# Aazmp/vp8oclenc

Hardware: AMD Instinct MI355X
Metric: macroblocks/sec inter-frame (ME+DCT+loopfilter), 1080p (higher is better)
Workload: dtype u8/int32

## Files before the change

vp8oclenc_amd/build.py:

```python
from __future__ import annotations

import os
import shutil
import subprocess

PKG = os.path.dirname(os.path.abspath(__file__))
CSRC = os.path.join(PKG, "csrc")
LIB = os.path.join(PKG, "libvp8hip.so")
SOURCES = ["api_context.hip", "api_intake.hip", "api_inter.hip", "api_entropy.hip", "api_batch.hip", "api_shard.hip", "api_profile.hip", "kernels_me.hip", "kernels_scale.hip", "kernels_denoise.hip", "api_denoise.hip", "kernels_analysis.hip", "api_analysis.hip", "kernels_convert.hip", "kernels_deinterlace.hip", "api_deinterlace.hip", "kernels_geometry.hip", "api_geometry.hip", "kernels_s2.hip", "kernels_mb.hip", "kernels_lf3.hip", "kernels_lf4.hip", "kernels_lf_simple.hip", "kernels_quality.hip", "api_quality.hip", "kernels_entropy_stage.hip", "kernels_rc.hip", "kernels_intra.hip", "vp8_host.cpp", "vp8_driver.cpp", "vp8_bitstream.cpp"]
HEADERS = ["vp8hip_ctx.h", "vp8hip_dev.h", "kernels_rc_dev.h", "lf_shared.h", "lf_banded.h", "lds_bank_model.h", "s1_pre_layout.h", "vp8_rfc6386_tables.inc", "vp8_mbhdr.h", "kernels_ent.hip", "kernels_hdr.hip"]
HEADERS = HEADERS + [os.path.join("..", "..", "include", h) for h in ("vp8hip.h", "vp8hip_multi.h", "vp8hip_taps.h", "vp8hip_host.h", "vp8hip_driver.h", "vp8hip_bitstream.h")]


def _hipcc() -> str:
    for cand in (shutil.which("hipcc"), "/opt/rocm/bin/hipcc"):
        if cand and os.path.exists(cand):
            return cand
    raise RuntimeError("hipcc not found: the MI355X path cannot be built (there is no CPU fallback)")


def stale() -> bool:
    if not os.path.exists(LIB):
        return True
    t = os.path.getmtime(LIB)
    deps = [os.path.join(CSRC, s) for s in SOURCES] + [os.path.normpath(os.path.join(CSRC, h)) for h in HEADERS]
    return any(os.path.exists(d) and os.path.getmtime(d) > t for d in deps)


def build(force: bool = False, verbose: bool = False) -> str:
    if not force and not stale():
        return LIB
    objs = []
    procs = []
    odir = os.path.join(PKG, "build")
    os.makedirs(odir, exist_ok=True)
    flags = ["--offload-arch=gfx950", "-O3", "-fPIC", "-std=c++17", "-ffp-contract=off", "-Wall", "-Wno-unused-function", "-Wno-bitwise-instead-of-logical", "-Wno-unused-value", "-Wno-missing-braces",
             "-I", os.path.join(PKG, "..", "include")] + os.environ.get("VP8HIP_EXTRA_FLAGS", "").split()
    for src in SOURCES:
        path = os.path.join(CSRC, src)
        if not os.path.exists(path):
            continue
        obj = os.path.join(odir, os.path.splitext(src)[0] + ".o")
        objs.append(obj)
# ... 20 lines not shown
```

vp8oclenc_amd/csrc/api_profile.hip:

```cpp
#include "vp8hip_ctx.h"

using namespace vp8;

namespace vp8 {

int prof_collect(vp8hip_ctx *c) {
    if (c->ev_used == 0) return VP8HIP_OK;
    HIPCHK(c, hipStreamSynchronize(c->stream));
    for (int i = 0; i < c->ev_used; i += 2) {
        float ms = 0;
        HIPCHK(c, hipEventElapsedTime(&ms, c->ev[i], c->ev[i + 1]));
        c->prof_ms[c->ev_kernel[i / 2]] += ms;
        c->prof_n[c->ev_kernel[i / 2]] += 1;
    }
    c->ev_used = 0;
    return VP8HIP_OK;
}

}

extern "C" {

int vp8hip_profile_enable(vp8hip_ctx *c, uint32_t mask) {
    USE_DEVICE(c);
// ... 109 lines not shown
    HIPCHK(c, hipStreamSynchronize(s));
    return VP8HIP_OK;
}

int vp8hip_debug_weight(vp8hip_ctx *c, const int32_t *d, int n, int32_t *out) {
    USE_DEVICE(c);
    JOIN_LF(c);
    if (!c || !d || !out || n <= 0) return VP8HIP_ERR_ARG;
    int32_t *dd = nullptr, *dout = nullptr;
    HIPCHK(c, hipMalloc(&dd, (size_t)n * 64));
    HIPCHK(c, hipMalloc(&dout, (size_t)n * 4));
    HIPCHK(c, hipMemcpyAsync(dd, d, (size_t)n * 64, hipMemcpyHostToDevice, c->stream));
    launch_weight_tap(c->stream, dd, n, dout);
    HIPCHK(c, hipMemcpyAsync(out, dout, (size_t)n * 4, hipMemcpyDeviceToHost, c->stream));
    HIPCHK(c, hipStreamSynchronize(c->stream));
    hipFree(dd);
    hipFree(dout);
    return VP8HIP_OK;
}

int vp8hip_debug_weight_mfma(vp8hip_ctx *c, const int32_t *d, int n, int32_t *out) {
    USE_DEVICE(c);
    JOIN_LF(c);
    if (!c || !d || !out || n <= 0) return VP8HIP_ERR_ARG;
    int32_t *dd = nullptr, *dout = nullptr;
    HIPCHK(c, hipMalloc(&dd, (size_t)n * 64));
    HIPCHK(c, hipMalloc(&dout, (size_t)n * 4));
    HIPCHK(c, hipMemcpyAsync(dd, d, (size_t)n * 64, hipMemcpyHostToDevice, c->stream));
    launch_weight_tap_mfma(c->stream, dd, n, dout);
    HIPCHK(c, hipMemcpyAsync(out, dout, (size_t)n * 4, hipMemcpyDeviceToHost, c->stream));
    HIPCHK(c, hipStreamSynchronize(c->stream));
    hipFree(dd);
    hipFree(dout);
    return VP8HIP_OK;
}

int vp8hip_debug_lf_stall(vp8hip_ctx *c, int on) {
    USE_DEVICE(c);
    JOIN_LF(c);
    if (!c) return VP8HIP_ERR_ARG;
    c->lf_stall_test = on ? 1 : 0;
    return VP8HIP_OK;
}

int vp8hip_debug_upload_ssim(vp8hip_ctx *c, const float *ssim) {
    USE_DEVICE(c);
    JOIN_LF(c);
    if (!c || !ssim) return VP8HIP_ERR_ARG;
    HIPCHK(c, hipMemcpyAsync(c->out.ssim, ssim, (size_t)c->mbs * 4, hipMemcpyHostToDevice, c->stream));
    HIPCHK(c, hipStreamSynchronize(c->stream));
    return VP8HIP_OK;
}

int vp8hip_debug_upload_header_inputs(vp8hip_ctx *c, const int32_t *seg, const int32_t *nz, const int32_t *ref, const int32_t *parts,
                                      const int16_t *vectors, const int32_t *is_inter, const int32_t *modes, const uint32_t *probs,
                                      const uint32_t *denom, const int32_t *sd) {
    USE_DEVICE(c);
    JOIN_LF(c);
    if (!c) return VP8HIP_ERR_ARG;
    hipStream_t s = c->stream;
    const size_t n = c->mbs;
    if (seg) HIPCHK(c, hipMemcpyAsync(c->out.seg, seg, n * 4, hipMemcpyHostToDevice, s));
    if (nz) HIPCHK(c, hipMemcpyAsync(c->out.nz, nz, n * 4, hipMemcpyHostToDevice, s));
    if (ref) HIPCHK(c, hipMemcpyAsync(c->out.ref, ref, n * 4, hipMemcpyHostToDevice, s));
    if (parts) HIPCHK(c, hipMemcpyAsync(c->out.parts, parts, n * 4, hipMemcpyHostToDevice, s));
    if (vectors) HIPCHK(c, hipMemcpyAsync(c->out.vec, vectors, n * 16, hipMemcpyHostToDevice, s));
// ... 12 lines not shown
```

vp8oclenc_amd/csrc/kernels_me.hip:

```cpp
#include <stdlib.h>
#include <string.h>

#include "vp8hip_dev.h"
#include "s1_pre_layout.h"

namespace vp8 {

struct BorderItem { Plane y, u, v; };
static_assert(EXT == 8, "border_row stores a margin as one eight-byte word");
__device__ __forceinline__ void border_row(const Plane &pl, int row, int lane) {
    if (row >= pl.h + EXT) return;
    uint8_t *dst = pl.p + (ptrdiff_t)row * pl.stride;
    const uint8_t *src = pl.p + (ptrdiff_t)iclamp(row, 0, pl.h - 1) * pl.stride;
    if (row < 0 || row >= pl.h)
        for (int x = lane * 8; x < pl.w; x += 512) *reinterpret_cast<uint2 *>(dst + x) = *reinterpret_cast<const uint2 *>(src + x);
    if (lane < 2) {
        const uint32_t s4 = (uint32_t)src[lane ? pl.w - 1 : 0] * 0x01010101u;
        *reinterpret_cast<uint2 *>(dst + (lane ? pl.w : -EXT)) = make_uint2(s4, s4);
    }
}
__device__ __forceinline__ void border_body(const BorderItem &a) {
    border_row(blockIdx.y == 0 ? a.y : (blockIdx.y == 1 ? a.u : a.v), (int)blockIdx.x - EXT, threadIdx.x);
}

__global__ __launch_bounds__(64) void k_border(BorderItem a) { border_body(a); }

void launch_border(hipStream_t s, const Frame &f) {
    dim3 grid(f.Y[0].h + 2 * EXT, 3);
    VP8_LAUNCH(k_border, grid, dim3(64), 0, s, BorderItem{f.Y[0], f.U, f.V});
}

struct PyrArgs { Frame f[2 * MAX_BATCH]; uint32_t border_mask; };
static int border_jobs(const Frame &f) { return (f.Y[0].h + 2 * EXT) + 2 * (f.U.h + 2 * EXT); }

__global__ __launch_bounds__(256) void k_pyramid(PyrArgs a) {
    __shared__ uint8_t s2[16][16];
    __shared__ uint8_t s3[8][8];
// ... 139 lines not shown
    int refmap[3];
    int nrefs;
    int net_width, w, h, pixel_rate, rate_shift, nblk, bw;
    int pbw, pbh;
    uint32_t bw_inv;
};

template <bool SPLIT>
struct S1Map {
    static constexpr int LANES_PER_BLOCK = SPLIT ? 20 : 5;
    static constexpr int BLOCKS_PER_WAVE = SPLIT ? 3 : 12;
    static constexpr int BLOCKS_PER_WG = 4 * BLOCKS_PER_WAVE;
};

__device__ __forceinline__ void s1_subblock(const uint8_t *cp, int cstride, const uint8_t *rp, int rstride, int acc[5]) {
    uint32_t c[4], q0[4], q1[4];
#pragma unroll
    for (int y = 0; y < 4; ++y) {
        c[y] = *reinterpret_cast<const uint32_t *>(cp + (ptrdiff_t)y * cstride) ^ 0x80808080u;
        const uint2 q = ld_u64(rp + (ptrdiff_t)y * rstride);
        q0[y] = q.x ^ 0x80808080u; q1[y] = q.y ^ 0x80808080u;
    }
    uint32_t cc[4], col[8];
    transpose4x4(c, cc);
    transpose4x4(q0, col);
    transpose4x4(q1, col + 4);
    int pre[16];
#pragma unroll
    for (int k = 0; k < 4; ++k) weight_pre_column(cc[k], pre + 4 * k);
#pragma unroll
    for (int i = 0; i < 5; ++i) acc[i] += weight_cols_pre(pre, col + i);
}

__device__ __forceinline__ int vcopy(uint32_t x) {
    int y;
    asm volatile("v_mov_b32 %0, %1" : "=v"(y) : "v"(x));
    return y;
}
__device__ __forceinline__ void s1_subblock_pre(v4i wa, const int *pre_lds, int pre_off, const uint8_t *rp, int rstride, int acc[5]) {
    uint32_t q0[4], q1[4];
#pragma unroll
    for (int y = 0; y < 4; ++y) {
        const uint2 q = ld_u64(rp + (ptrdiff_t)y * rstride);
        q0[y] = q.x ^ 0x80808080u; q1[y] = q.y ^ 0x80808080u;
    }
    uint32_t col[8];
    transpose4x4(q0, col);
    transpose4x4(q1, col + 4);
#pragma unroll
    for (int i = 0; i < 5; ++i) {
        int off = pre_off;
        asm volatile("" : "+v"(off));
        __builtin_amdgcn_sched_barrier(0);
        const v4i b = (i & 1) ? v4i{vcopy(col[i]), vcopy(col[i + 1]), vcopy(col[i + 2]), vcopy(col[i + 3])}
                              : v4i{(int)col[i], (int)col[i + 1], (int)col[i + 2], (int)col[i + 3]};
        acc[i] += weight_mfma(wa, load_pre16(pre_lds + off), b);
    }
}
static_assert(s1_pre_c_read_worst() == 4 && s1_pre_c_read_best() == 4, "the C reads of the whole-pel search's pre table must be free of LDS bank conflicts");
static_assert(S1_PRE_BLOCKS == S1Map<false>::BLOCKS_PER_WAVE, "s1_pre_layout.h and the loop form's lane map disagree");
__device__ __forceinline__ void s1_make_pre(const Plane &cur, int cx, int cy, int sb, bool on, int *dst16) {
    const int sx = (sb >> 1) * 4, sy = (sb & 1) * 4;
    const uint8_t *cp = cur.p + (ptrdiff_t)(cy + sy) * cur.stride + cx + sx;
    uint32_t c[4], cc[4];
#pragma unroll
    for (int y = 0; y < 4; ++y) c[y] = *reinterpret_cast<const uint32_t *>(cp + (ptrdiff_t)y * cur.stride) ^ 0x80808080u;
    transpose4x4(c, cc);
    int pre[16];
    weight_pre_block(cc, pre);
    if (on) {
#pragma unroll
        for (int k = 0; k < 4; ++k) *reinterpret_cast<int4 *>(dst16 + 4 * k) = make_int4(pre[4 * k], pre[4 * k + 1], pre[4 * k + 2], pre[4 * k + 3]);
    }
}

template <bool SPLIT, bool PRE_LDS = false>
__device__ __forceinline__ uint32_t search1_block(const Search1Args &a, int r, int cx, int cy, uint32_t pv, bool live, int sub, int lane,
                                                  const int *pre_lds = nullptr ,
                                                  int pre_off = 0 ) {
    const int sb0 = sub / 5, j = sub - 5 * sb0;
    int v0x = (int16_t)(pv & 0xffffu), v0y = (int16_t)(pv >> 16);
    const int rmask = a.pixel_rate - 1;
    v0x = (v0x + ((v0x >> 31) & rmask)) >> a.rate_shift;
    v0y = (v0y + ((v0y >> 31) & rmask)) >> a.rate_shift;
    if (a.pixel_rate > 8) v0x = v0y = 0;

    const int py = (int16_t)(cy + v0y + (j - 2));
    const bool row_valid = live && py >= 0 && py <= a.h - 8;
    const int xb = cx + v0x - 2;
    const bool loadable = row_valid && xb >= -8 && xb <= a.w - 4;
    const int lx = loadable ? xb : cx, ly = loadable ? py : cy;

    const uint8_t *cp = a.cur.p + (ptrdiff_t)cy * a.cur.stride + cx;
    const uint8_t *rp = a.ref[r].p + (ptrdiff_t)ly * a.ref[r].stride + lx;
    int acc[5] = {0, 0, 0, 0, 0};
    if (SPLIT) {
        const int sx = (sb0 >> 1) * 4, sy = (sb0 & 1) * 4;
        s1_subblock(cp + (ptrdiff_t)sy * a.cur.stride + sx, a.cur.stride, rp + (ptrdiff_t)sy * a.ref[r].stride + sx, a.ref[r].stride, acc);
#pragma unroll
        for (int i = 0; i < 5; ++i) {
            acc[i] += __shfl(acc[i], lane + 10, 64);
            acc[i] += __shfl(acc[i], lane + 5, 64);
        }
    } else {
        if (PRE_LDS) {
            const v4i wa = metric_a(lane);
#pragma unroll 1
            for (int sb = 0; sb < 4; ++sb) {
                const int sx = (sb >> 1) * 4, sy = (sb & 1) * 4;
                s1_subblock_pre(wa, pre_lds, pre_off + s1_pre_sub_at(sb), rp + (ptrdiff_t)sy * a.ref[r].stride + sx, a.ref[r].stride, acc);
            }
        } else {
#pragma unroll 1
            for (int sb = 0; sb < 4; ++sb) {
                const int sx = (sb >> 1) * 4, sy = (sb & 1) * 4;
                s1_subblock(cp + (ptrdiff_t)sy * a.cur.stride + sx, a.cur.stride, rp + (ptrdiff_t)sy * a.ref[r].stride + sx, a.ref[r].stride, acc);
            }
        }
    }
    const int pen_mask = a.pixel_rate < 4 ? -1 : 0;
    const int pen_y = iabs(iabs(py - cy) - v0y);
    uint32_t best = 0xffffffffu;
#pragma unroll
    for (int i = 0; i < 5; ++i) {
        const int px = (int16_t)(xb + i);
        const bool valid = loadable && px >= 0 && px <= a.w - 8;
        const int diff = (acc[i] + (((iabs(iabs(px - cx) - v0x) + pen_y) << 5) & pen_mask)) & 0xffff;
        const uint32_t key = (valid && diff < 0x7fff) ? ((uint32_t)diff << 8) | (uint32_t)(j * 5 + i) : 0xffffffffu;
        best = key < best ? key : best;
    }
#pragma unroll
    for (int off = 1; off <= 4; off <<= 1) {
        const uint32_t o = (uint32_t)__shfl((int)best, lane + off, 64);
        if (j + off < 5 && o < best) best = o;
    }
    int bx, by;
    if (best != 0xffffffffu) {
        const int k = best & 0xff;
        bx = v0x + (k % 5 - 2);
        by = v0y + (k / 5 - 2);
    } else {
        bx = (int16_t)(v0x - cx);
        by = (int16_t)(v0y - cy);
    }
    const uint32_t ox16 = (uint16_t)(int16_t)((int16_t)bx * (int16_t)a.pixel_rate);
    const uint32_t oy16 = (uint16_t)(int16_t)((int16_t)by * (int16_t)a.pixel_rate);
    return ox16 | (oy16 << 16);
}

template <bool SPLIT, bool PRE_LDS = false, bool REF_LOOP = false>
__device__ __forceinline__ void search1_body(const Search1Args &a) {
    using M = S1Map<SPLIT>;
    if (!REF_LOOP && (int)blockIdx.y >= a.nrefs) return;
    const int lane = threadIdx.x & 63, wave = threadIdx.x >> 6;
    const int grp = lane / M::LANES_PER_BLOCK, sub = lane - M::LANES_PER_BLOCK * grp;
    const int b_raw = (xcd_band(blockIdx.x, gridDim.x) * 4 + wave) * M::BLOCKS_PER_WAVE + grp;
    const bool live = grp < M::BLOCKS_PER_WAVE && b_raw < a.nblk;
    const int b = live ? b_raw : a.nblk - 1;
    const int by = a.bw == 1 ? b : (int)__umulhi((uint32_t)b, a.bw_inv), bx = b - by * a.bw;
    const int cx = bx * 8, cy = by * 8;
    const int parent = (cy >> 4) * a.net_width + (cx >> 4);
    const bool parent_written = (cx >> 4) < a.pbw && (cy >> 4) < a.pbh;
    const int *pre_lds = nullptr;
    int pre_off = 0;
    if (!SPLIT && PRE_LDS) {
        __shared__ __attribute__((aligned(16))) int s_pre[4][S1_PRE_INTS];
        const int slot = lane >> 2, sb = lane & 3;
        const int tb_raw = (xcd_band(blockIdx.x, gridDim.x) * 4 + wave) * M::BLOCKS_PER_WAVE + slot;
        const int tb = tb_raw < a.nblk ? tb_raw : a.nblk - 1;
        const int tby = a.bw == 1 ? tb : (int)__umulhi((uint32_t)tb, a.bw_inv), tbx = tb - tby * a.bw;
        s1_make_pre(a.cur, tbx * 8, tby * 8, sb, slot < M::BLOCKS_PER_WAVE, &s_pre[0][0] + s1_pre_slot_at(wave, slot) + s1_pre_sub_at(sb));
        asm volatile("s_waitcnt lgkmcnt(0)" ::: "memory");
        pre_lds = &s_pre[0][0];
        pre_off = s1_pre_c_at(wave, lane, 0, 0);
    }
    const int nr = REF_LOOP ? a.nrefs : 1;
#pragma unroll 1
    for (int ri = 0; ri < nr; ++ri) {
        const int r = a.refmap[REF_LOOP ? ri : (int)blockIdx.y];
        const uint32_t pv = parent_written ? reinterpret_cast<const uint32_t *>(a.src[r])[parent] : 0u;
        const uint32_t out = search1_block<SPLIT, !SPLIT && PRE_LDS>(a, r, cx, cy, pv, live, sub, lane, pre_lds, pre_off);
        if (sub == 0 && live) {
            const int cell = (cy >> 3) * a.net_width + (cx >> 3);
            reinterpret_cast<uint32_t *>(a.dst[r])[cell] = out;
        }
    }
}

struct CoarseArgs { Search1Args lv[5]; };
constexpr int COARSE_WAVES = 6;
template <bool FINEST, bool TOP_ONLY = false>
__device__ __forceinline__ void coarse_tile(const Search1Args &L0, const Search1Args &L1, const Search1Args &L2, const Search1Args &L3, const Search1Args &L4, int r) {
    using M = S1Map<true>;
    __shared__ uint32_t mv4, mv3, mv2[4], mv1[16];
    const int lane = threadIdx.x & 63, wave = threadIdx.x >> 6;
    const int grp = lane / M::LANES_PER_BLOCK, sub = lane - M::LANES_PER_BLOCK * grp;
    const int slot = grp < M::BLOCKS_PER_WAVE ? wave * M::BLOCKS_PER_WAVE + grp : 99;
    const int tiles_x = (L1.bw + 3) / 4;
    const int tile = xcd_band(blockIdx.x, gridDim.x);
    const int ty = tile / tiles_x, tx = tile - ty * tiles_x;
    {
        const int bx = tx >> 1, by = ty >> 1;
        const bool exists = bx < L4.bw && by * L4.bw + bx < L4.nblk;
        if (wave == 0) {
            const bool live = slot == 0 && exists;
            const uint32_t out = search1_block<true>(L4, r, (live ? bx : 0) * 8, (live ? by : 0) * 8, 0u, live, sub, lane);
            if (slot == 0 && sub == 0) mv4 = exists ? out : 0u;
        }
    }
    __syncthreads();
    {
        const bool exists = tx < L3.bw && ty * L3.bw + tx < L3.nblk;
        if (wave == 0) {
            const bool live = slot == 0 && exists;
// ... 60 lines not shown
    s.net_width = a.net_width;
    s.w = g.w;
    s.h = g.h;
    s.pixel_rate = 1 << l;
    s.rate_shift = l;
    s.bw = g.w / 8;
    s.nblk = (g.w / 8) * (g.h / 8);
    return s;
}
__global__ __launch_bounds__(128) void k_search1_top_b(CoarseBatchArgs a) {
    const CoarseMember &m = a.m[blockIdx.z];
    if ((int)blockIdx.y >= m.nrefs) return;
    const int r = m.refmap[blockIdx.y];
    const Search1Args L1 = coarse_level(a, m, 1, r), L2 = coarse_level(a, m, 2, r), L3 = coarse_level(a, m, 3, r), L4 = coarse_level(a, m, 4, r);
    coarse_tile<false, true>(L1, L1, L2, L3, L4, 0);
}
template <bool FINEST>
__global__ __launch_bounds__(64 * COARSE_WAVES) void k_search1_coarse_b(CoarseBatchArgs a) {
    const CoarseMember &m = a.m[blockIdx.z];
    if ((int)blockIdx.y >= m.nrefs) return;
    const int r = m.refmap[blockIdx.y];
    const Search1Args L0 = coarse_level(a, m, 0, r), L1 = coarse_level(a, m, 1, r), L2 = coarse_level(a, m, 2, r), L3 = coarse_level(a, m, 3, r),
                      L4 = coarse_level(a, m, 4, r);
    coarse_tile<FINEST>(L0, L1, L2, L3, L4, 0);
}

template <bool SPLIT>
__global__ __launch_bounds__(256) void k_search1(Search1Args a) { search1_body<SPLIT>(a); }
static_assert(sizeof(BatchOf<Search1Args>) <= 4096 && sizeof(PyrArgs) <= 4096 && sizeof(BatchOf<PackItem>) <= 4096, "a batch's argument blocks travel in the 4 KiB kernel-argument segment");
template <bool SPLIT>
__global__ __launch_bounds__(256) void k_search1_b(BatchOf<Search1Args> b) { search1_body<SPLIT>(b.item[blockIdx.z]); }
__global__ __attribute__((amdgpu_waves_per_eu(8, 8))) __launch_bounds__(256) void k_search1_pl(Search1Args a) { search1_body<false, true>(a); }
__global__ __attribute__((amdgpu_waves_per_eu(8, 8))) __launch_bounds__(256) void k_search1_pl_b(BatchOf<Search1Args> b) { search1_body<false, true>(b.item[blockIdx.z]); }
__global__ __attribute__((amdgpu_waves_per_eu(7, 8))) __launch_bounds__(256) void k_search1_plr_b(BatchOf<Search1Args> b) { search1_body<false, true, true>(b.item[blockIdx.z]); }
static bool search1_ref_loop() {
    static const bool on = [] { const char *v = getenv("VP8HIP_S1_REF_LOOP"); return !(v && v[0] == '0'); }();
    return on;
}
static bool search1_pre_lds() {
    static const bool on = [] { const char *v = getenv("VP8HIP_S1_PRE_LDS"); return !(v && v[0] == '0'); }();
    return on;
}

static Search1Args search1_args(const CodingItem &it, int level, int src_idx, int net_width) {
    const Frame &cur = *it.cur;
    const RefSet &refs = it.refs;
    const NetSet &nets = *it.nets;
    Search1Args a;
    a.cur = cur.Y[level];
    int n = 0;
    for (int r = 0; r < 3; ++r) {
        a.ref[r] = refs.ref[r].Y[level];
        a.src[r] = nets.net[r][src_idx];
        a.dst[r] = nets.net[r][src_idx ^ 1];
        if (refs.use[r]) a.refmap[n++] = r;
    }
    a.nrefs = n;
    for (int i = n; i < 3; ++i) a.refmap[i] = 0;
    a.net_width = net_width;
    a.w = a.cur.w;
    a.h = a.cur.h;
    a.pixel_rate = 1 << level;
    a.rate_shift = level;
    a.bw = a.w / 8;
    a.nblk = (a.w / 8) * (a.h / 8);
    a.bw_inv = a.bw > 0 ? (uint32_t)(((1ull << 32) + a.bw - 1) / a.bw) : 0;
    a.pbw = level < 4 ? cur.Y[level + 1].w / 8 : 0;
// ... 64 lines not shown
            if (refs.use[r]) m.refmap[k++] = r;
        }
        m.nrefs = k;
        for (int j = k; j < 3; ++j) m.refmap[j] = 0;
        maxrefs = k > maxrefs ? k : maxrefs;
    }
    const int bw0 = a.g[0].w / 8, bh0 = a.g[0].h / 8, bw1 = a.g[1].w / 8, bh1 = a.g[1].h / 8;
    if (bw0 * bh0 <= 0 || maxrefs == 0 || search1_skip()) return true;
    const int tiles_x = finest ? (bw0 + 7) / 8 : (bw1 + 3) / 4, tiles_y = finest ? (bh0 + 7) / 8 : (bh1 + 3) / 4;
    if (tiles_x * tiles_y <= 0) return !finest ? true : false;
    if (top_only) {
        VP8_LAUNCH(k_search1_top_b, dim3(tiles_x * tiles_y, maxrefs, n), dim3(128), 0, s, a);
        return true;
    }
    if (finest) VP8_LAUNCH(k_search1_coarse_b<true>, dim3(tiles_x * tiles_y, maxrefs, n), dim3(64 * COARSE_WAVES), 0, s, a);
    else VP8_LAUNCH(k_search1_coarse_b<false>, dim3(tiles_x * tiles_y, maxrefs, n), dim3(64 * COARSE_WAVES), 0, s, a);
    return true;
}

void launch_search1_batch(hipStream_t s, const CodingItem *items, int n, int level, int src_idx, int net_width) {
    BatchOf<Search1Args> b;
    b.n = n;
    int maxrefs = 0, totrefs = 0;
    for (int i = 0; i < n; ++i) {
        b.item[i] = search1_args(items[i], level, src_idx, net_width);
        maxrefs = b.item[i].nrefs > maxrefs ? b.item[i].nrefs : maxrefs;
        totrefs += b.item[i].nrefs;
    }
    const int nblk = b.item[0].nblk;
    if (nblk <= 0 || maxrefs == 0 || search1_skip()) return;
    if (search1_split((size_t)nblk * totrefs, false))
        VP8_LAUNCH(k_search1_b<true>, dim3((nblk + S1Map<true>::BLOCKS_PER_WG - 1) / S1Map<true>::BLOCKS_PER_WG, maxrefs, n), dim3(256), 0, s, b);
    else if (search1_pre_lds() && search1_ref_loop())
        VP8_LAUNCH(k_search1_plr_b, dim3((nblk + S1Map<false>::BLOCKS_PER_WG - 1) / S1Map<false>::BLOCKS_PER_WG, 1, n), dim3(256), 0, s, b);
    else if (search1_pre_lds())
        VP8_LAUNCH(k_search1_pl_b, dim3((nblk + S1Map<false>::BLOCKS_PER_WG - 1) / S1Map<false>::BLOCKS_PER_WG, maxrefs, n), dim3(256), 0, s, b);
    else
        VP8_LAUNCH(k_search1_b<false>, dim3((nblk + S1Map<false>::BLOCKS_PER_WG - 1) / S1Map<false>::BLOCKS_PER_WG, maxrefs, n), dim3(256), 0, s, b);
}

__global__ __launch_bounds__(256) void k_weight_tap(const int32_t *d, int n, int32_t *out) {
    const int i = blockIdx.x * 256 + threadIdx.x;
    if (i >= n) return;
    uint32_t cc[4], pp[4];
#pragma unroll
    for (int c = 0; c < 4; ++c) {
        cc[c] = pp[c] = 0;
#pragma unroll
        for (int r = 0; r < 4; ++r) {
            const int v = d[i * 16 + 4 * r + c];
            const uint32_t cb = (uint32_t)(v > 0 ? v : 0) ^ 0x80u, pb = (uint32_t)(v > 0 ? 0 : -v) ^ 0x80u;
            cc[c] |= cb << (8 * r);
            pp[c] |= pb << (8 * r);
        }
    }
    int pre[16];
#pragma unroll
    for (int c = 0; c < 4; ++c) weight_pre_column(cc[c], pre + 4 * c);
    out[i] = weight_cols_pre(pre, pp);
}
void launch_weight_tap(hipStream_t s, const int32_t *d, int n, int32_t *out) {
    hipLaunchKernelGGL(k_weight_tap, dim3((n + 255) / 256), dim3(256), 0, s, d, n, out);
}
__global__ __attribute__((amdgpu_waves_per_eu(8, 8))) __launch_bounds__(256) void k_weight_tap_mfma(const int32_t *d, int n, int32_t *out) {
    const int i0 = blockIdx.x * 256 + threadIdx.x, i = i0 < n ? i0 : n - 1;
    uint32_t cc[4];
    v4i pp;
#pragma unroll
    for (int c = 0; c < 4; ++c) {
        uint32_t cw = 0, pw = 0;
#pragma unroll
        for (int r = 0; r < 4; ++r) {
            const int v = d[i * 16 + 4 * r + c];
            const uint32_t cb = (uint32_t)(v > 0 ? v : 0) ^ 0x80u, pb = (uint32_t)(v > 0 ? 0 : -v) ^ 0x80u;
            cw |= cb << (8 * r);
            pw |= pb << (8 * r);
        }
        cc[c] = cw;
        pp[c] = (int)pw;
    }
    int pre[16];
    weight_pre_block(cc, pre);
    v16i c16;
#pragma unroll
    for (int k = 0; k < 16; ++k) c16[k] = pre[k];
    const int w = weight_mfma(metric_a((int)threadIdx.x), c16, pp);
    if (i0 < n) out[i0] = w;
}
void launch_weight_tap_mfma(hipStream_t s, const int32_t *d, int n, int32_t *out) {
    hipLaunchKernelGGL(k_weight_tap_mfma, dim3((n + 255) / 256), dim3(256), 0, s, d, n, out);
}

}
```

vp8oclenc_amd/csrc/vp8hip_dev.h:

```cpp
#pragma once
#include <hip/hip_runtime.h>
#include <hip/hip_ext.h>
#include <stdint.h>
#include <stdlib.h>
#include <string.h>

#include <vector>

#include "../../include/vp8hip.h"

namespace vp8 {

struct LaunchTiming { hipEvent_t start = nullptr, stop = nullptr; int launches = 0; };
extern thread_local LaunchTiming tl_timing;
#define VP8_LAUNCH(kernel, grid, block, shmem, stream, ...)                                                                               \
    do {                                                                                                                                  \
        ++::vp8::tl_timing.launches;                                                                                                      \
        hipExtLaunchKernelGGL(kernel, grid, block, shmem, stream, ::vp8::tl_timing.start, ::vp8::tl_timing.stop, 0, __VA_ARGS__);         \
    } while (0)

constexpr int PAD = 32;
constexpr int EXT = 8;
constexpr int LF_ERR_WORD = 1536;
constexpr int LF_SIMPLE_WORD = 512;
// ... 127 lines not shown
    int32_t *verdict;
    uint32_t seq;
};
struct CodingItem {
    const Frame *cur;
    RefSet refs;
    const NetSet *nets;
    const Frame *recon;
    const MBOut *out;
    const SegData *sd;
    const ScanRequest *scan;
};
struct FilterItem {
    const Frame *recon;
    const MBOut *out;
    SegData *sd;
    int32_t *progress;
    void *handoff;
    unsigned launch_no;
    LfCheck chk;
};
bool launch_search1_coarse_batch(hipStream_t s, const CodingItem *items, int n, int net_width, bool finest, bool top_only = false);
void launch_search1_batch(hipStream_t s, const CodingItem *items, int n, int level, int src_idx, int net_width);
bool launch_search2_batch(hipStream_t s, const CodingItem *items, int n, unsigned long long *clk = nullptr);
void launch_mb_batch(hipStream_t s, const CodingItem *items, int n, float ssim_target, int mbw, int mbh, bool conformant = false);
void launch_loop_filter3_batch(hipStream_t s, const FilterItem *items, int n, int mbw, int mbh);
void launch_loop_filter4_batch(hipStream_t s, const FilterItem *items, int n, int mbw, int mbh);
void launch_auto_segments_batch(hipStream_t s, const ScanRequest *q, int n);
void launch_search1_coarse(hipStream_t s, const CodingItem &it, int net_width, bool finest);
void launch_search1(hipStream_t s, const CodingItem &it, int level, int src_idx, int net_width, bool latency = false);
void launch_search2(hipStream_t s, const CodingItem &it, unsigned long long *clk = nullptr);
void launch_weight_tap(hipStream_t s, const int32_t *d, int n, int32_t *out);
void launch_weight_tap_mfma(hipStream_t s, const int32_t *d, int n, int32_t *out);
void launch_filter_mask(hipStream_t s, const MBOut &o, const SegData *d_sd, int mbs);
void launch_loop_filter4(hipStream_t s, const FilterItem &it, int mbw, int mbh, int stall_test = 0);
size_t loop_filter4_handoff_bytes(int mbw, int mbh);
void launch_loop_filter_simple(hipStream_t s, const FilterItem &it, int mbw, int mbh);
void launch_loop_filter_simple_batch(hipStream_t s, const FilterItem *items, int n, int mbw, int mbh);
bool loop_filter_simple_fits(int mbh);

constexpr int QUALITY_TILE_COLS = 63;
constexpr int QUALITY_TILE_ROWS = 8;
struct QualitySums {
    int64_t frames;
    uint64_t sse[3], samples[3];
    double psnr_all_sum, ssim_all_sum, ssim_sum[3], psnr_min;
    int64_t psnr_min_frame;
};
struct QualityState {
    vp8hip_quality pending;
    int32_t has_pending;
    uint32_t seq;
    QualitySums sums;
};
struct QualityPartial { unsigned long long sse; double ssim; };
struct QualityPlane { const uint8_t *s, *r; int ss, rs, w, h; };
struct QualityArgs {
    QualityPlane p[3];
    QualityPartial *partial;
    unsigned *ticket;
    QualityState *state;
    QualityState *host;
    uint32_t seq;
    int32_t frame_number, is_key;
};
int quality_tiles(int w, int h);
// ... 236 lines not shown
        const int t3 = dot2(xy, K_ROT16_B, 16 * 7500);
        A[c] = as_s16x2(__builtin_amdgcn_perm((uint32_t)t1, (uint32_t)R0, 0x07060100u));
        B[c] = as_s16x2(__builtin_amdgcn_perm((uint32_t)t3, (uint32_t)R2, 0x07060100u));
    }
    return weight_rows(A, B);
}

typedef int v4i __attribute__((ext_vector_type(4)));
typedef int v16i __attribute__((ext_vector_type(16)));
enum { METRIC_S0, METRIC_M0, METRIC_C0, METRIC_D0, METRIC_S2, METRIC_M2, METRIC_C2, METRIC_D2, METRIC_X , METRIC_Y = 12  };
constexpr uint32_t metric_w(int i, int c) {
    if (i >= METRIC_X) return (i & 3) != c ? 0u : i >= METRIC_Y ? K_W_YN : K_W_XN;
    const uint32_t pos = i < METRIC_S2 ? K_W_R0N : K_W_R2N, neg = i < METRIC_S2 ? K_W_R0 : K_W_R2;
    switch (i & 3) {
    case METRIC_S0: return pos;
    case METRIC_M0: return c == 0 || c == 3 ? pos : neg;
    case METRIC_C0: return c == 1 ? pos : c == 2 ? neg : 0u;
    default: return c == 0 ? pos : c == 3 ? neg : 0u;
    }
}
struct MetricTable { uint32_t w[64][4]; };
constexpr MetricTable make_metric_a() {
    MetricTable t{};
    for (int l = 0; l < 64; ++l) {
        const int m = l & 31, h = l >> 5;
        if (((m >> 2) & 1) != h) continue;
        const int i = (m & 3) + 4 * (m >> 3);
        for (int c = 0; c < 4; ++c) t.w[l][c] = metric_w(i, c);
    }
    return t;
}
static __device__ __constant__ const MetricTable K_METRIC_A = make_metric_a();
__device__ __forceinline__ v4i metric_a(int wave_lane) { return *reinterpret_cast<const v4i *>(K_METRIC_A.w[wave_lane & 63]); }

__device__ __forceinline__ void weight_pre_half(const uint32_t cc[4], uint32_t k_r, uint32_t k_xy, int smcd[4], int xy[4]) {
    int R[4];
#pragma unroll
    for (int c = 0; c < 4; ++c) {
        R[c] = dot4s(cc[c], k_r, 0);
        xy[c] = dot4s(cc[c], k_xy, 0);
    }
    const int a7 = R[0] + R[3] + 0x8007, b = R[1] + R[2];
    smcd[METRIC_S0] = a7 + b;
    smcd[METRIC_M0] = a7 - b;
    smcd[METRIC_C0] = R[1] - R[2];
    smcd[METRIC_D0] = R[0] - R[3];
}
__device__ __forceinline__ void weight_pre_block(const uint32_t cc[4], int pre[16]) {
    weight_pre_half(cc, K_W_R0, K_W_X, pre + METRIC_S0, pre + METRIC_X);
    weight_pre_half(cc, K_W_R2, K_W_Y, pre + METRIC_S2, pre + METRIC_Y);
}

__device__ __forceinline__ int weight_mfma(v4i a, v16i c, v4i p) {
    const v16i d = __builtin_amdgcn_mfma_i32_32x32x32_i8(a, p, c, 0, 0, 0);
    s16x2 P[4];
#pragma unroll
    for (int col = 0; col < 4; ++col) {
        const uint32_t xy = pk16(d[METRIC_X + col], d[METRIC_Y + col]);
        const int t1 = dot2(xy, K_ROT16_A, 16 * 14500);
        const int t3 = dot2(xy, K_ROT16_B, 16 * 7500);
        P[col] = as_s16x2(__builtin_amdgcn_perm((uint32_t)t3, (uint32_t)t1, 0x07060302u));
    }
    uint32_t acc = 0;
    {
        const s16x2 a1 = P[0] + P[3], d1 = P[0] - P[3], b1 = P[1] + P[2], c1 = P[1] - P[2];
        const u16x2 a7 = __builtin_bit_cast(u16x2, a1) + u16x2{0x8007, 0x8007};
// ... 51 lines not shown
```

Measured before the change: 73.24 million.

## Pack search1 ref-loop workgroups with 51 blocks of 5 lanes and row-major MFMA operands

The default ref-loop search1 kernel now packs 51 five-lane blocks into each 256-thread workgroup instead of a per-wave mapping. It builds one shared pre table for the whole workgroup with a skewed layout checked by static asserts to be free of LDS bank conflicts, and it finds the per-block minimum through LDS with a barrier instead of shuffles. The MFMA weight operand is transposed into a row-major table, so reference rows can feed the B operand through alignbyte without a 4x4 transpose and copy. This raises lane utilisation and removes transpose work, but adds a __syncthreads per reference and more LDS traffic. It also adds debug entry points for testing.

Result: faster. 74.35 million (median of 6 runs) (+1.5%).

```diff
diff --git a/vp8oclenc_amd/build.py b/vp8oclenc_amd/build.py
--- a/vp8oclenc_amd/build.py
+++ b/vp8oclenc_amd/build.py
@@ -8,7 +8,7 @@
 CSRC = os.path.join(PKG, "csrc")
 LIB = os.path.join(PKG, "libvp8hip.so")
 SOURCES = ["api_context.hip", "api_intake.hip", "api_inter.hip", "api_entropy.hip", "api_batch.hip", "api_shard.hip", "api_profile.hip", "kernels_me.hip", "kernels_scale.hip", "kernels_denoise.hip", "api_denoise.hip", "kernels_analysis.hip", "api_analysis.hip", "kernels_convert.hip", "kernels_deinterlace.hip", "api_deinterlace.hip", "kernels_geometry.hip", "api_geometry.hip", "kernels_s2.hip", "kernels_mb.hip", "kernels_lf3.hip", "kernels_lf4.hip", "kernels_lf_simple.hip", "kernels_quality.hip", "api_quality.hip", "kernels_entropy_stage.hip", "kernels_rc.hip", "kernels_intra.hip", "vp8_host.cpp", "vp8_driver.cpp", "vp8_bitstream.cpp"]
-HEADERS = ["vp8hip_ctx.h", "vp8hip_dev.h", "kernels_rc_dev.h", "lf_shared.h", "lf_banded.h", "lds_bank_model.h", "s1_pre_layout.h", "vp8_rfc6386_tables.inc", "vp8_mbhdr.h", "kernels_ent.hip", "kernels_hdr.hip"]
+HEADERS = ["vp8hip_ctx.h", "vp8hip_dev.h", "kernels_rc_dev.h", "lf_shared.h", "lf_banded.h", "lds_bank_model.h", "s1_pre_layout.h", "s1_fill_layout.h", "vp8_rfc6386_tables.inc", "vp8_mbhdr.h", "kernels_ent.hip", "kernels_hdr.hip"]
 HEADERS = HEADERS + [os.path.join("..", "..", "include", h) for h in ("vp8hip.h", "vp8hip_multi.h", "vp8hip_taps.h", "vp8hip_host.h", "vp8hip_driver.h", "vp8hip_bitstream.h")]
 
 
diff --git a/vp8oclenc_amd/csrc/api_profile.hip b/vp8oclenc_amd/csrc/api_profile.hip
--- a/vp8oclenc_amd/csrc/api_profile.hip
+++ b/vp8oclenc_amd/csrc/api_profile.hip
@@ -165,6 +165,57 @@
     HIPCHK(c, hipStreamSynchronize(c->stream));
     hipFree(dd);
     hipFree(dout);
+    return VP8HIP_OK;
+}
+
+int vp8hip_debug_weight_mfma_rows(vp8hip_ctx *c, const int32_t *d, int n, int32_t *out) {
+    USE_DEVICE(c);
+    JOIN_LF(c);
+    if (!c || !d || !out || n <= 0) return VP8HIP_ERR_ARG;
+    int32_t *dd = nullptr, *dout = nullptr;
+    HIPCHK(c, hipMalloc(&dd, (size_t)n * 64));
+    HIPCHK(c, hipMalloc(&dout, (size_t)n * 4));
+    HIPCHK(c, hipMemcpyAsync(dd, d, (size_t)n * 64, hipMemcpyHostToDevice, c->stream));
+    launch_weight_tap_mfma_rows(c->stream, dd, n, dout);
+    HIPCHK(c, hipMemcpyAsync(out, dout, (size_t)n * 4, hipMemcpyDeviceToHost, c->stream));
+    HIPCHK(c, hipStreamSynchronize(c->stream));
+    hipFree(dd);
+    hipFree(dout);
+    return VP8HIP_OK;
+}
+
+int vp8hip_debug_search1_batch(vp8hip_ctx *const *ctxs, int n, const int *use_golden, const int *use_altref, int level,
+                               const int16_t *const *src, int16_t *const *dst) {
+    if (!ctxs || n <= 0 || n > MAX_BATCH || !use_golden || !use_altref || level < 0 || level > 4 || !src || !dst) return VP8HIP_ERR_ARG;
+    vp8hip_ctx *c0 = ctxs[0];
+    USE_DEVICE(c0);
+    CodingItem it[MAX_BATCH];
+    for (int i = 0; i < n; ++i) {
+        vp8hip_ctx *c = ctxs[i];
+        if (!c || c->b8 != c0->b8 || c->mbw != c0->mbw) return VP8HIP_ERR_ARG;
+        JOIN_LF(c);
+        it[i] = coding_item(c, use_golden[i], use_altref[i]);
+        for (int r = 0; r < 3; ++r) {
+            if (!it[i].refs.use[r]) continue;
+            if (!src[3 * i + r] || !dst[3 * i + r]) return VP8HIP_ERR_ARG;
+            HIPCHK(c0, hipMemcpyAsync(c->nets.net[r][0], src[3 * i + r], (size_t)c->b8 * 4, hipMemcpyHostToDevice, c0->stream));
+            HIPCHK(c0, hipMemsetAsync(c->nets.net[r][1], 0, (size_t)c->b8 * 4, c0->stream));
+        }
+    }
+    launch_search1_batch(c0->stream, it, n, level, 0, c0->mbw * 2);
+    for (int i = 0; i < n; ++i)
+        for (int r = 0; r < 3; ++r)
+            if (it[i].refs.use[r]) HIPCHK(c0, hipMemcpyAsync(dst[3 * i + r], ctxs[i]->nets.net[r][1], (size_t)ctxs[i]->b8 * 4, hipMemcpyDeviceToHost, c0->stream));
+    HIPCHK(c0, hipStreamSynchronize(c0->stream));
+    HIPCHK(c0, hipGetLastError());
+    return VP8HIP_OK;
+}
+
+int vp8hip_debug_metric_tables(uint32_t *a_cols, uint32_t *a_rows) {
+    if (!a_cols || !a_rows) return VP8HIP_ERR_ARG;
+    static constexpr MetricTable cols = make_metric_a(), rows = make_metric_a_rows();
+    memcpy(a_cols, cols.w, sizeof(cols.w));
+    memcpy(a_rows, rows.w, sizeof(rows.w));
     return VP8HIP_OK;
 }
 
diff --git a/vp8oclenc_amd/csrc/kernels_me.hip b/vp8oclenc_amd/csrc/kernels_me.hip
--- a/vp8oclenc_amd/csrc/kernels_me.hip
+++ b/vp8oclenc_amd/csrc/kernels_me.hip
@@ -3,6 +3,7 @@
 
 #include "vp8hip_dev.h"
 #include "s1_pre_layout.h"
+#include "s1_fill_layout.h"
 
 namespace vp8 {
 
@@ -208,28 +209,21 @@
     for (int i = 0; i < 5; ++i) acc[i] += weight_cols_pre(pre, col + i);
 }
 
-__device__ __forceinline__ int vcopy(uint32_t x) {
-    int y;
-    asm volatile("v_mov_b32 %0, %1" : "=v"(y) : "v"(x));
-    return y;
-}
 __device__ __forceinline__ void s1_subblock_pre(v4i wa, const int *pre_lds, int pre_off, const uint8_t *rp, int rstride, int acc[5]) {
     uint32_t q0[4], q1[4];
 #pragma unroll
     for (int y = 0; y < 4; ++y) {
-        const uint2 q = ld_u64(rp + (ptrdiff_t)y * rstride);
-        q0[y] = q.x ^ 0x80808080u; q1[y] = q.y ^ 0x80808080u;
-    }
-    uint32_t col[8];
-    transpose4x4(q0, col);
-    transpose4x4(q1, col + 4);
+        q0[y] = ld_u32(rp + (ptrdiff_t)y * rstride) ^ 0x80808080u;
+        q1[y] = ld_u32(rp + (ptrdiff_t)y * rstride + 4) ^ 0x80808080u;
+    }
 #pragma unroll
     for (int i = 0; i < 5; ++i) {
         int off = pre_off;
         asm volatile("" : "+v"(off));
         __builtin_amdgcn_sched_barrier(0);
-        const v4i b = (i & 1) ? v4i{vcopy(col[i]), vcopy(col[i + 1]), vcopy(col[i + 2]), vcopy(col[i + 3])}
-                              : v4i{(int)col[i], (int)col[i + 1], (int)col[i + 2], (int)col[i + 3]};
+        v4i b;
+#pragma unroll
+        for (int y = 0; y < 4; ++y) b[y] = i == 0 ? (int)q0[y] : i == 4 ? (int)q1[y] : (int)__builtin_amdgcn_alignbyte(q1[y], q0[y], (uint32_t)i);
         acc[i] += weight_mfma(wa, load_pre16(pre_lds + off), b);
     }
 }
@@ -250,10 +244,11 @@
     }
 }
 
-template <bool SPLIT, bool PRE_LDS = false>
+template <bool SPLIT, bool PRE_LDS = false, bool LDS_MIN = false>
 __device__ __forceinline__ uint32_t search1_block(const Search1Args &a, int r, int cx, int cy, uint32_t pv, bool live, int sub, int lane,
                                                   const int *pre_lds = nullptr ,
-                                                  int pre_off = 0 ) {
+                                                  int pre_off = 0 ,
+                                                  uint32_t *min_lds = nullptr ) {
     const int sb0 = sub / 5, j = sub - 5 * sb0;
     int v0x = (int16_t)(pv & 0xffffu), v0y = (int16_t)(pv >> 16);
     const int rmask = a.pixel_rate - 1;
@@ -280,7 +275,7 @@
         }
     } else {
         if (PRE_LDS) {
-            const v4i wa = metric_a(lane);
+            const v4i wa = metric_a_rows(lane);
 #pragma unroll 1
             for (int sb = 0; sb < 4; ++sb) {
                 const int sx = (sb >> 1) * 4, sy = (sb & 1) * 4;
@@ -305,10 +300,20 @@
         const uint32_t key = (valid && diff < 0x7fff) ? ((uint32_t)diff << 8) | (uint32_t)(j * 5 + i) : 0xffffffffu;
         best = key < best ? key : best;
     }
-#pragma unroll
-    for (int off = 1; off <= 4; off <<= 1) {
-        const uint32_t o = (uint32_t)__shfl((int)best, lane + off, 64);
-        if (j + off < 5 && o < best) best = o;
+    if (LDS_MIN) {
+        min_lds[sub] = best;
+        __syncthreads();
+#pragma unroll
+        for (int k = 0; k < 5; ++k) {
+            const uint32_t o = min_lds[k];
+            best = o < best ? o : best;
+        }
+    } else {
+#pragma unroll
+        for (int off = 1; off <= 4; off <<= 1) {
+            const uint32_t o = (uint32_t)__shfl((int)best, lane + off, 64);
+            if (j + off < 5 && o < best) best = o;
+        }
     }
     int bx, by;
     if (best != 0xffffffffu) {
@@ -324,14 +329,18 @@
     return ox16 | (oy16 << 16);
 }
 
-template <bool SPLIT, bool PRE_LDS = false, bool REF_LOOP = false>
+static_assert(s1_fill_c_read_worst() == 4 && s1_fill_c_read_best() == 4, "the C reads of the filled loop form's pre table must be free of LDS bank conflicts: all four waves, every sub-block and quad");
+static_assert(s1_fill_c_read_worst(64) > 4, "the bank model sees the conflicts of unskewed slots");
+template <bool SPLIT, bool PRE_LDS = false, bool REF_LOOP = false, bool FILL = false>
 __device__ __forceinline__ void search1_body(const Search1Args &a) {
     using M = S1Map<SPLIT>;
+    static_assert(!FILL || (!SPLIT && PRE_LDS && REF_LOOP), "the filled map is the loop form's, with the table in LDS and the reference loop");
     if (!REF_LOOP && (int)blockIdx.y >= a.nrefs) return;
     const int lane = threadIdx.x & 63, wave = threadIdx.x >> 6;
-    const int grp = lane / M::LANES_PER_BLOCK, sub = lane - M::LANES_PER_BLOCK * grp;
-    const int b_raw = (xcd_band(blockIdx.x, gridDim.x) * 4 + wave) * M::BLOCKS_PER_WAVE + grp;
-    const bool live = grp < M::BLOCKS_PER_WAVE && b_raw < a.nblk;
+    const int grp = FILL ? s1_fill_slot_of((int)threadIdx.x) : lane / M::LANES_PER_BLOCK;
+    const int sub = FILL ? (int)threadIdx.x - S1_FILL_LANES * grp : lane - M::LANES_PER_BLOCK * grp;
+    const int b_raw = FILL ? s1_fill_block_of(xcd_band(blockIdx.x, gridDim.x), grp, a.nblk) : (xcd_band(blockIdx.x, gridDim.x) * 4 + wave) * M::BLOCKS_PER_WAVE + grp;
+    const bool live = FILL ? b_raw >= 0 : grp < M::BLOCKS_PER_WAVE && b_raw < a.nblk;
     const int b = live ? b_raw : a.nblk - 1;
     const int by = a.bw == 1 ? b : (int)__umulhi((uint32_t)b, a.bw_inv), bx = b - by * a.bw;
     const int cx = bx * 8, cy = by * 8;
@@ -339,7 +348,20 @@
     const bool parent_written = (cx >> 4) < a.pbw && (cy >> 4) < a.pbh;
     const int *pre_lds = nullptr;
     int pre_off = 0;
-    if (!SPLIT && PRE_LDS) {
+    uint32_t *min_lds = nullptr;
+    if (FILL) {
+        __shared__ __attribute__((aligned(16))) int s_fill[S1_FILL_INTS];
+        __shared__ uint32_t s_min[2][S1_FILL_MIN_WORDS];
+        const int t = threadIdx.x, slot = s1_fill_task_slot(t), sb = s1_fill_task_sub(t);
+        const int tb_raw = xcd_band(blockIdx.x, gridDim.x) * S1_FILL_BLOCKS + slot;
+        const int tb = tb_raw < a.nblk ? tb_raw : a.nblk - 1;
+        const int tby = a.bw == 1 ? tb : (int)__umulhi((uint32_t)tb, a.bw_inv), tbx = tb - tby * a.bw;
+        s1_make_pre(a.cur, tbx * 8, tby * 8, sb, slot < S1_FILL_BLOCKS, s_fill + s1_fill_slot_at(slot) + s1_pre_sub_at(sb));
+        __syncthreads();
+        pre_lds = s_fill;
+        pre_off = s1_fill_c_at(t, 0, 0);
+        min_lds = &s_min[0][s1_fill_min_at(t)];
+    } else if (!SPLIT && PRE_LDS) {
         __shared__ __attribute__((aligned(16))) int s_pre[4][S1_PRE_INTS];
         const int slot = lane >> 2, sb = lane & 3;
         const int tb_raw = (xcd_band(blockIdx.x, gridDim.x) * 4 + wave) * M::BLOCKS_PER_WAVE + slot;
@@ -355,7 +377,8 @@
     for (int ri = 0; ri < nr; ++ri) {
         const int r = a.refmap[REF_LOOP ? ri : (int)blockIdx.y];
         const uint32_t pv = parent_written ? reinterpret_cast<const uint32_t *>(a.src[r])[parent] : 0u;
-        const uint32_t out = search1_block<SPLIT, !SPLIT && PRE_LDS>(a, r, cx, cy, pv, live, sub, lane, pre_lds, pre_off);
+        const uint32_t out = search1_block<SPLIT, !SPLIT && PRE_LDS, FILL>(a, r, cx, cy, pv, live, sub, lane, pre_lds, pre_off,
+                                                                            FILL ? min_lds + (ri & 1) * S1_FILL_MIN_WORDS : nullptr);
         if (sub == 0 && live) {
             const int cell = (cy >> 3) * a.net_width + (cx >> 3);
             reinterpret_cast<uint32_t *>(a.dst[r])[cell] = out;
@@ -482,7 +505,7 @@
 __global__ __launch_bounds__(256) void k_search1_b(BatchOf<Search1Args> b) { search1_body<SPLIT>(b.item[blockIdx.z]); }
 __global__ __attribute__((amdgpu_waves_per_eu(8, 8))) __launch_bounds__(256) void k_search1_pl(Search1Args a) { search1_body<false, true>(a); }
 __global__ __attribute__((amdgpu_waves_per_eu(8, 8))) __launch_bounds__(256) void k_search1_pl_b(BatchOf<Search1Args> b) { search1_body<false, true>(b.item[blockIdx.z]); }
-__global__ __attribute__((amdgpu_waves_per_eu(7, 8))) __launch_bounds__(256) void k_search1_plr_b(BatchOf<Search1Args> b) { search1_body<false, true, true>(b.item[blockIdx.z]); }
+__global__ __attribute__((amdgpu_waves_per_eu(7, 8))) __launch_bounds__(256) void k_search1_plr_b(BatchOf<Search1Args> b) { search1_body<false, true, true, true>(b.item[blockIdx.z]); }
 static bool search1_ref_loop() {
     static const bool on = [] { const char *v = getenv("VP8HIP_S1_REF_LOOP"); return !(v && v[0] == '0'); }();
     return on;
@@ -613,7 +636,7 @@
     if (search1_split((size_t)nblk * totrefs, false))
         VP8_LAUNCH(k_search1_b<true>, dim3((nblk + S1Map<true>::BLOCKS_PER_WG - 1) / S1Map<true>::BLOCKS_PER_WG, maxrefs, n), dim3(256), 0, s, b);
     else if (search1_pre_lds() && search1_ref_loop())
-        VP8_LAUNCH(k_search1_plr_b, dim3((nblk + S1Map<false>::BLOCKS_PER_WG - 1) / S1Map<false>::BLOCKS_PER_WG, 1, n), dim3(256), 0, s, b);
+        VP8_LAUNCH(k_search1_plr_b, dim3(s1_fill_grid(nblk), 1, n), dim3(256), 0, s, b);
     else if (search1_pre_lds())
         VP8_LAUNCH(k_search1_pl_b, dim3((nblk + S1Map<false>::BLOCKS_PER_WG - 1) / S1Map<false>::BLOCKS_PER_WG, maxrefs, n), dim3(256), 0, s, b);
     else
@@ -671,5 +694,32 @@
 void launch_weight_tap_mfma(hipStream_t s, const int32_t *d, int n, int32_t *out) {
     hipLaunchKernelGGL(k_weight_tap_mfma, dim3((n + 255) / 256), dim3(256), 0, s, d, n, out);
 }
-
-}
+__global__ __attribute__((amdgpu_waves_per_eu(8, 8))) __launch_bounds__(256) void k_weight_tap_mfma_rows(const int32_t *d, int n, int32_t *out) {
+    const int i0 = blockIdx.x * 256 + threadIdx.x, i = i0 < n ? i0 : n - 1;
+    uint32_t cc[4] = {0, 0, 0, 0};
+    v4i pp = {0, 0, 0, 0};
+#pragma unroll
+    for (int r = 0; r < 4; ++r) {
+        uint32_t pw = 0;
+#pragma unroll
+        for (int c = 0; c < 4; ++c) {
+            const int v = d[i * 16 + 4 * r + c];
+            const uint32_t cb = (uint32_t)(v > 0 ? v : 0) ^ 0x80u, pb = (uint32_t)(v > 0 ? 0 : -v) ^ 0x80u;
+            cc[c] |= cb << (8 * r);
+            pw |= pb << (8 * c);
+        }
+        pp[r] = (int)pw;
+    }
+    int pre[16];
+    weight_pre_block(cc, pre);
+    v16i c16;
+#pragma unroll
+    for (int k = 0; k < 16; ++k) c16[k] = pre[k];
+    const int w = weight_mfma(metric_a_rows((int)threadIdx.x), c16, pp);
+    if (i0 < n) out[i0] = w;
+}
+void launch_weight_tap_mfma_rows(hipStream_t s, const int32_t *d, int n, int32_t *out) {
+    hipLaunchKernelGGL(k_weight_tap_mfma_rows, dim3((n + 255) / 256), dim3(256), 0, s, d, n, out);
+}
+
+}
diff --git a/vp8oclenc_amd/csrc/s1_fill_layout.h b/vp8oclenc_amd/csrc/s1_fill_layout.h
--- /dev/null
+++ b/vp8oclenc_amd/csrc/s1_fill_layout.h
@@ -0,0 +1,49 @@
+#pragma once
+#include "s1_pre_layout.h"
+
+constexpr int S1_FILL_LANES = 5;
+constexpr int S1_FILL_BLOCKS = 51;
+constexpr int S1_FILL_INTS = S1_FILL_BLOCKS * S1_PRE_SLOT;
+constexpr int S1_FILL_MIN_WORDS = 256 + S1_FILL_LANES - 1;
+
+LDS_MODEL_HD constexpr int s1_fill_slot_of(int t) { return t / S1_FILL_LANES; }
+LDS_MODEL_HD constexpr int s1_fill_sub_of(int t) { return t % S1_FILL_LANES; }
+LDS_MODEL_HD constexpr int s1_fill_grid(int nblk) { return (nblk + S1_FILL_BLOCKS - 1) / S1_FILL_BLOCKS; }
+LDS_MODEL_HD constexpr int s1_fill_block_of(int tile, int slot, int nblk) {
+    return slot < S1_FILL_BLOCKS && tile * S1_FILL_BLOCKS + slot < nblk ? tile * S1_FILL_BLOCKS + slot : -1;
+}
+LDS_MODEL_HD constexpr int s1_fill_min_at(int t) { return t - s1_fill_sub_of(t); }
+LDS_MODEL_HD constexpr int s1_fill_slot_at(int slot, int slot_ints = S1_PRE_SLOT) { return (slot < S1_FILL_BLOCKS ? slot : S1_FILL_BLOCKS - 1) * slot_ints; }
+LDS_MODEL_HD constexpr int s1_fill_task_slot(int t) { return t >> 2; }
+LDS_MODEL_HD constexpr int s1_fill_task_sub(int t) { return t & 3; }
+LDS_MODEL_HD constexpr int s1_fill_c_at(int t, int sb, int j, int slot_ints = S1_PRE_SLOT) {
+    return s1_fill_slot_at(s1_fill_slot_of(t), slot_ints) + s1_pre_sub_at(sb, j);
+}
+
+LDS_MODEL_HD constexpr int s1_fill_c_read_cycles(int wave, int sb, int j, int slot_ints = S1_PRE_SLOT, unsigned long long exec = ~0ull) {
+    lds_model::WaveAddrs w{};
+    for (int l = 0; l < 64; ++l) w.a[l] = 4u * (unsigned)s1_fill_c_at(64 * wave + l, sb, j, slot_ints);
+    return lds_model::ds_read_b128_cycles(w, exec);
+}
+LDS_MODEL_HD constexpr int s1_fill_c_read_worst(int slot_ints = S1_PRE_SLOT, unsigned long long exec = ~0ull) {
+    int worst = 0;
+    for (int wave = 0; wave < 4; ++wave)
+        for (int sb = 0; sb < 4; ++sb)
+            for (int j = 0; j < 4; ++j) {
+                const int c = s1_fill_c_read_cycles(wave, sb, j, slot_ints, exec);
+                worst = c > worst ? c : worst;
+            }
+    return worst;
+}
+LDS_MODEL_HD constexpr int s1_fill_c_read_best(int slot_ints = S1_PRE_SLOT, unsigned long long exec = ~0ull) {
+    int best = 1 << 30;
+    for (int wave = 0; wave < 4; ++wave)
+        for (int sb = 0; sb < 4; ++sb)
+            for (int j = 0; j < 4; ++j) {
+                const int c = s1_fill_c_read_cycles(wave, sb, j, slot_ints, exec);
+                best = c < best ? c : best;
+            }
+    return best;
+}
+static_assert(S1_FILL_BLOCKS * S1_FILL_LANES <= 256 && (S1_FILL_BLOCKS + 1) * S1_FILL_LANES > 256, "as many whole blocks as a workgroup of 256 lanes holds");
+static_assert(4 * S1_FILL_BLOCKS <= 256, "the workgroup makes its table in one pass: a lane per (slot, sub-block)");
diff --git a/vp8oclenc_amd/csrc/vp8hip_dev.h b/vp8oclenc_amd/csrc/vp8hip_dev.h
--- a/vp8oclenc_amd/csrc/vp8hip_dev.h
+++ b/vp8oclenc_amd/csrc/vp8hip_dev.h
@@ -183,6 +183,7 @@
 void launch_search2(hipStream_t s, const CodingItem &it, unsigned long long *clk = nullptr);
 void launch_weight_tap(hipStream_t s, const int32_t *d, int n, int32_t *out);
 void launch_weight_tap_mfma(hipStream_t s, const int32_t *d, int n, int32_t *out);
+void launch_weight_tap_mfma_rows(hipStream_t s, const int32_t *d, int n, int32_t *out);
 void launch_filter_mask(hipStream_t s, const MBOut &o, const SegData *d_sd, int mbs);
 void launch_loop_filter4(hipStream_t s, const FilterItem &it, int mbw, int mbh, int stall_test = 0);
 size_t loop_filter4_handoff_bytes(int mbw, int mbh);
@@ -485,6 +486,19 @@
 }
 static __device__ __constant__ const MetricTable K_METRIC_A = make_metric_a();
 __device__ __forceinline__ v4i metric_a(int wave_lane) { return *reinterpret_cast<const v4i *>(K_METRIC_A.w[wave_lane & 63]); }
+constexpr MetricTable make_metric_a_rows() {
+    MetricTable t{};
+    for (int l = 0; l < 64; ++l) {
+        const int m = l & 31, h = l >> 5;
+        if (((m >> 2) & 1) != h) continue;
+        const int i = (m & 3) + 4 * (m >> 3);
+        for (int r = 0; r < 4; ++r)
+            for (int c = 0; c < 4; ++c) t.w[l][r] |= ((metric_w(i, c) >> (8 * r)) & 255u) << (8 * c);
+    }
+    return t;
+}
+static __device__ __constant__ const MetricTable K_METRIC_A_ROWS = make_metric_a_rows();
+__device__ __forceinline__ v4i metric_a_rows(int wave_lane) { return *reinterpret_cast<const v4i *>(K_METRIC_A_ROWS.w[wave_lane & 63]); }
 
 __device__ __forceinline__ void weight_pre_half(const uint32_t cc[4], uint32_t k_r, uint32_t k_xy, int smcd[4], int xy[4]) {
     int R[4];
```
